# pszenher/Distributional_RL_Decision_and_Control

Hardware: AMD Instinct MI355X
Metric: env-steps/sec/GPU @4096 envs; IQN learn-steps/sec at 1/2/4/8 GPUs (higher is better)
Workload: dtype f64-env/bf16-learner; 1 GPU; BASELINE config 2: 4096 envs x 5 robots, 4 buoys, 55m map; fused rollout + AC-IQN learn (B=4096, N=N'=32) per step; envs_per_gpu=4096, robots=5, obstacles=4, global_batch=4096, num_tau=32, parallelism=dp1, hip_graphs=True, dp_rehearsal=False, unroll=2, chained=True, fused_reset=True, env_groups=0, target_after_env=False, push_after_actor=True, target_in_fused=True

## Files before the change

distributional_rl_decision_and_control_amd/_abi.py:

```python
import ctypes as C
import os

import numpy as np

HERE = os.path.dirname(os.path.abspath(__file__))
LIB_PATH = os.environ.get("ASVRL_LIB", os.path.join(HERE, "lib", "libasvrl.so"))
LIB_PATH_F32 = os.path.join(HERE, "lib", "libasvrl_f32.so")
OPERANDS = {"bf16": (LIB_PATH, 2), "f32": (LIB_PATH_F32, 4)}
ABI_VERSION = 29

SELF_DIM, OBJ_DIM, MAX_OBJ = 7, 5, 5
OBS_DIM = 40
TR_DIM = 88
PER_DIM = 48

F_X, F_Y, F_THETA, F_VR0, F_VR1, F_VR2, F_V0, F_V1, F_V2, F_TL, F_TR, F_LP, F_RP, F_GX, F_GY, F_PHI, F_RET = range(17)
NUM_FIELDS = 17

FLAG_DEACTIVATED, FLAG_COLLISION, FLAG_REACH_GOAL, FLAG_COLREGS = 1, 2, 4, 8

INFO_NORMAL, INFO_TOO_LONG, INFO_COLLISION, INFO_REACH_GOAL, INFO_DEACT_COLLISION, INFO_DEACT_GOAL = range(6)
INFO_ABSENT = 255
INFO_STRINGS = {
    INFO_NORMAL: "normal",
# ... 339 lines not shown
    ("asvrl_linear_wgrad_vec_groups", _I32, [_I32]),
    ("asvrl_linear_wgrad_partial", C.c_int, [_VP, _I64, _VP, _I64, _I32, _I32, _I32, _VP, _I64, _VP, _VP]),
    ("asvrl_linear_wgrad_multi", C.c_int, [_VP, _I32, _VP, _VP]),
    ("asvrl_linear_wgrad_vec_partial", C.c_int, [_VP, _I64, _VP, _I64, _I32, _I32, _VP, _I64, _VP, _VP]),
    ("asvrl_small_wgrad_partial", C.c_int, [_VP, _I64, _VP, _I64, _I32, _I32, _I32, _VP, _I64, _VP, _VP]),
    ("asvrl_partial_sums", C.c_int, [_VP, _I32, _VP]),
    ("asvrl_partial_sums_norm", C.c_int, [_VP, _I32, _VP, _VP, _VP]),
    ("asvrl_partial_sums_norm_parts", _I32, [_VP, _I32]),
    ("asvrl_actor_grads_workspace", _I64, [_I32]),
    ("asvrl_actor_grads_counters", _I32, []),
    ("asvrl_actor_grads_norm_parts", _I32, []),
    ("asvrl_actor_grads", C.c_int, [C.POINTER(AsvActorGradIO), _VP]),
    ("asvrl_adam_step", C.c_int, [_VP, _VP, _VP, _VP, _I64, _VP, _F, _F, _F, _F, _F, _VP, _VP, _I32, _VP]),
    ("asvrl_adam_step_pack", C.c_int, [_VP, _VP, _VP, _VP, _I64, _VP, _F, _F, _F, _F, _F, _VP, _VP, _I32, _VP, _I32,
                                       _VP, _VP]),
    ("asvrl_linear_wgrad", C.c_int, [_VP, _I64, _VP, _I64, _I32, _I32, _I32, _VP, _VP, _I32, _VP, _I64, _VP]),
    ("asvrl_linear_wgrad_vec", C.c_int, [_VP, _I64, _VP, _I64, _I32, _I32, _VP, _VP, _I32, _VP, _I64, _VP]),
    ("asvrl_mlp_pack", C.c_int, [C.POINTER(AsvMlpSrc), C.POINTER(AsvMlpWeights), _VP]),
    ("asvrl_mlp_encode", C.c_int, [C.POINTER(AsvMlpWeights), C.POINTER(AsvMlpIO), _VP]),
    ("asvrl_actor_forward", C.c_int, [C.POINTER(AsvMlpWeights), C.POINTER(AsvMlpIO), _I32, _VP]),
    ("asvrl_actor_backward", C.c_int, [C.POINTER(AsvMlpWeights), C.POINTER(AsvMlpIO), _VP]),
    ("asvrl_learn_prologue", C.c_int, [C.POINTER(AsvSampleArgs), C.POINTER(AsvMlpWeights), C.POINTER(AsvMlpIO),
                                       C.POINTER(AsvMlpWeights), _VP, _VP]),
    ("asvrl_encoder_fold", C.c_int, [_VP, _VP, _VP, _VP, _VP, _VP, _I32, _VP]),
    ("asvrl_small_wgrad", C.c_int, [_VP, _I64, _VP, _I64, _I32, _I32, _I32, _VP, _VP, _I32, _VP, _I64, _VP]),
    ("asvrl_last_error", C.c_char_p, []),
    ("asvrl_abi_version", C.c_int, []),
    ("asvrl_operand_bytes", C.c_int32, []),
    ("asvrl_struct_sizes", None, [C.c_void_p]),
    ("asvrl_rollout_struct_size", _I64, []),
    ("asvrl_policy_rollout", C.c_int, [C.POINTER(AsvParams), C.POINTER(AsvEnvState), C.POINTER(AsvStepCtl),
                                       C.POINTER(AsvStepOut), C.POINTER(AsvRollout), C.POINTER(AsvPolicy),
                                       C.POINTER(AsvEnvLaunch), _VP]),
    ("asvrl_policy_struct_size", _I64, []),
    ("asvrl_env_rollout_ar", C.c_int, [C.POINTER(AsvParams), C.POINTER(AsvEnvState), C.POINTER(AsvStepCtl),
                                       C.POINTER(AsvStepOut), C.POINTER(AsvRollout), C.POINTER(AsvAutoReset),
                                       C.POINTER(AsvEnvLaunch), _VP]),
    ("asvrl_policy_rollout_ar", C.c_int, [C.POINTER(AsvParams), C.POINTER(AsvEnvState), C.POINTER(AsvStepCtl),
                                          C.POINTER(AsvStepOut), C.POINTER(AsvRollout), C.POINTER(AsvPolicy),
                                          C.POINTER(AsvAutoReset), C.POINTER(AsvEnvLaunch), _VP]),
    ("asvrl_autoreset_struct_size", _I64, []),
    ("asvrl_replay_push_window", C.c_int, [_VP, _VP, _VP, _VP, _I32, _I64, _VP, _VP, _I32, _I32, _VP, _VP, _I64, _VP,
                                           _VP, _VP, _VP, _I64, _VP]),
    ("asvrl_eval_metrics", C.c_int, [C.POINTER(AsvEvalMetrics), _VP]),
    ("asvrl_eval_metrics_struct_size", _I64, []),
    ("asvrl_dqn_pack", C.c_int, [C.POINTER(AsvMlpSrc), _VP, C.POINTER(AsvDqnWeights), _VP]),
# ... 130 lines not shown
```

distributional_rl_decision_and_control_amd/csrc/asvrl_mlp.hip:

```cpp
#include "asvrl_common.h"
#include "asvrl_mfma.h"
#include "asvrl_lds.h"
#include "asvrl_actor_tile.h"

namespace asvrl {
namespace {
using namespace atile;

template <int KS, int P>
__device__ __forceinline__ f32x16 wchain(const frag8* W, int base, int lane, const elem_t* img, const RowA<P>& RA) {
  f32x16 acc = f32x16{};
#pragma unroll
  for (int ks = 0; ks < KS; ++ks) acc = mfma(W[(base + ks) * 64 + lane], rowf(img, RA, 0, ks), acc);
  return acc;
}

constexpr int kMlpWaves = 4;

__global__ __launch_bounds__(kMlpWaves * 64) void encode_kernel(MlpArgs a) {
  const int lane = threadIdx.x & 63, h = lane >> 5, r = lane & 31;
  const int tile = blockIdx.x * kMlpWaves + (threadIdx.x >> 6);
  const AsvMlpIO& io = a.io;
  if (tile * 32 >= io.n) return;
  const int row = tile * 32 + r;
  const bool valid = row < io.n;
  const int rr = valid ? row : io.n - 1;
// ... 145 lines not shown
  for (int ks = 0; ks < kEnc / 16; ++ks) q.w1[ks] = W1[(w * 16 + ks) * 64 + lane];
#pragma unroll
  for (int ks = 0; ks < kHid / 16; ++ks) q.w2[ks] = W2[(w * 8 + ks) * 64 + lane];
}

__device__ __forceinline__ void bias16(const float* tab, int mb, int h, float (&b)[16]) {
  typedef float f4v __attribute__((ext_vector_type(4)));
#pragma unroll
  for (int k = 0; k < 4; ++k) {
    const f4v t = *reinterpret_cast<const f4v*>(tab + mb * 32 + 8 * k + 4 * h);
#pragma unroll
    for (int i = 0; i < 4; ++i) b[4 * k + i] = t[i];
  }
}

static_assert(kSelfF >= 32 && kObjF >= 32, "a 32-feature block spans at most two encoders");
__device__ __forceinline__ float obj_sel(int ob, const float (&mf)[kObjN]) {
  float f = 1.f;
#pragma unroll
  for (int o = 0; o < kObjN; ++o) f = ob == o ? mf[o] : f;
  return f;
}

template <int MODE, bool PRE = false>
__device__ __forceinline__ void actor_split_tile(const MlpArgs& a, ActorSplitLds& L, int tile, const float* x,
                                                 int64_t ldx, int xrow0, const SplitPre& pre = SplitPre{}) {
  const AsvMlpIO& io = a.io;
  const int lane = threadIdx.x & 63, w = __builtin_amdgcn_readfirstlane(threadIdx.x >> 6), h = lane >> 5,
            r = lane & 31;
  const int row = tile * 32 + r;
  const bool valid = row < io.n;
  const int rr = valid ? row : io.n - 1;
  {
    frag8 bx[2];
    float mk[kObjN];
    load_obs(x, ldx, xrow0 + (rr - tile * 32), h, bx, mk);
    PRO_STAMP(10);
    if (MODE == MLP_TRAIN && w == 0 && valid) {
#pragma unroll
      for (int ks = 0; ks < 2; ++ks)
        *reinterpret_cast<frag8*>(bp(io.xb) + static_cast<int64_t>(row) * kObsK + ks * 16 + 8 * h) = bx[ks];
    }
    const frag8* ENC = reinterpret_cast<const frag8*>(a.w.enc_frag);
    const RowA<kEnc> RA(r, h);
    float mf[kObjN];
#pragma unroll
    for (int o = 0; o < kObjN; ++o) mf[o] = mk[o] < 0.5f ? 0.f : 1.f;
#pragma unroll
    for (int q = 0; q < 2; ++q) {
      const int mb = 2 * w + q;
      float bb[16];
      bias16(L.bias + kSbEnc, mb, h, bb);
      const int m_lo = mb * 32;
      const int obA = m_lo < kSelfF ? -1 : obj_of(m_lo);
      const int lim = kSelfF + kObjF * (obA + 1) - m_lo - 4 * h;
      const float fA = obj_sel(obA, mf), fB = obj_sel(obA + 1, mf);
      f32x16 acc = f32x16{};
#pragma unroll
      for (int ks = 0; ks < 2; ++ks)
        acc = mfma(PRE ? pre.enc[2 * q + ks] : ENC[(mb * 2 + ks) * 64 + lane], bx[ks], acc);
#pragma unroll
      for (int s = 0; s < 2; ++s) {
        float v[8];
#pragma unroll
        for (int j = 0; j < 8; ++j) {
          const int g = 8 * s + j;
          v[j] = relu(acc[g] + bb[g]) * ((g & 3) + 8 * (g >> 2) < lim ? fA : fB);
        }
        rows(L.x0, RA, 0, 2 * mb + s, pack8(v));
        if constexpr (MODE == MLP_TRAIN)
          store16(valid ? bp(io.h0) + static_cast<int64_t>(row) * kEnc + mb * 32 + 16 * s : nullptr, v, h);
      }
      if (q == 0) PRO_STAMP(11);
    }
  }
  PRO_STAMP(5);
  __syncthreads();
  PRO_STAMP(6);
  {
    const frag8* W1 = reinterpret_cast<const frag8*>(a.w.w1_frag);
    const RowA<kEnc> RX(r, h);
    const RowA<kHid> RH(r, h);
    float bb[16];
    bias16(L.bias + kSbB1, w, h, bb);
    f32x16 acc = f32x16{};
    if constexpr (PRE) {
#pragma unroll
      for (int ks = 0; ks < kEnc / 16; ++ks) acc = mfma(pre.w1[ks], rowf(L.x0, RX, 0, ks), acc);
    } else {
      acc = wchain<kEnc / 16>(W1, w * 16, lane, L.x0, RX);
    }
#pragma unroll
    for (int s = 0; s < 2; ++s) {
      float v[8];
#pragma unroll
      for (int j = 0; j < 8; ++j) v[j] = relu(acc[8 * s + j] + bb[8 * s + j]);
      rows(L.h1, RH, 0, 2 * w + s, pack8(v));
      if constexpr (MODE == MLP_TRAIN)
        store16(valid ? bp(io.h1) + static_cast<int64_t>(row) * kHid + w * 32 + 16 * s : nullptr, v, h);
    }
  }
  PRO_STAMP(7);
  __syncthreads();
  {
    const frag8* W2 = reinterpret_cast<const frag8*>(a.w.w2_frag);
    const RowA<kHid> RH(r, h);
    float bb[16], wo0[16], wo1[16];
    bias16(L.bias + kSbB2, w, h, bb);
    bias16(L.bias + kSbWout, w, h, wo0);
    bias16(L.bias + kSbWout + kHid, w, h, wo1);
    f32x16 acc = f32x16{};
    if constexpr (PRE) {
#pragma unroll
      for (int ks = 0; ks < kHid / 16; ++ks) acc = mfma(pre.w2[ks], rowf(L.h1, RH, 0, ks), acc);
    } else {
      acc = wchain<kHid / 16>(W2, w * 8, lane, L.h1, RH);
    }
    float p0 = 0.f, p1 = 0.f;
#pragma unroll
    for (int s = 0; s < 2; ++s) {
      float v[8];
#pragma unroll
      for (int j = 0; j < 8; ++j) {
        v[j] = relu(acc[8 * s + j] + bb[8 * s + j]);
        p0 += wo0[8 * s + j] * v[j];
        p1 += wo1[8 * s + j] * v[j];
      }
// ... 27 lines not shown
template <int MODE>
__global__ __launch_bounds__(kMlpWaves * 64) void actor_split_kernel(MlpArgs a) {
  __shared__ __attribute__((aligned(16))) ActorSplitLds L;
  SplitPre pre;
  split_prefetch(a.w, threadIdx.x >> 6, threadIdx.x & 63, pre);
  float bv[4];
  split_bias_fetch(a.w, threadIdx.x, bv);
  split_bias_store(L, threadIdx.x, bv);
  __syncthreads();
  actor_split_tile<MODE, true>(a, L, blockIdx.x, a.io.x, a.io.ldx, blockIdx.x * 32, pre);
}

struct PrologueArgs {
  const float* ring;
  int64_t cap;
  const int64_t* ring_state;
  uint64_t seed, counter;
  const uint64_t* counter_dev;
  int64_t guard;
  int B, tau_sets, tau_n;
  float* out;
  float* taus;
};

__global__ __launch_bounds__(kMlpWaves * 64) void learn_prologue_kernel(PrologueArgs p, MlpArgs train, MlpArgs tgt) {
  PRO_STAMP(0);
  __shared__ __attribute__((aligned(16))) ActorSplitLds L;
  __shared__ __attribute__((aligned(16))) float xs[32 * ASVRL_OBS_DIM];
  const int T = p.B / 32;
  const bool second = static_cast<int>(blockIdx.x) >= T;
  const int tile = second ? blockIdx.x - T : blockIdx.x;
  const int lane = threadIdx.x & 63, w = threadIdx.x >> 6;
  SplitPre pre;
  split_prefetch(second ? tgt.w : train.w, w, lane, pre);
  float bv[4];
  split_bias_fetch(second ? tgt.w : train.w, threadIdx.x, bv);
  const int64_t head = p.ring_state[0], size = p.ring_state[1];
  const uint64_t ctr = p.counter + (p.counter_dev != nullptr ? *p.counter_dev : 0ull);
  const int64_t my_slot = replay_draw_slot(head, size, p.cap, p.guard, tile * 32 + 8 * w + (lane & 7), p.seed, ctr);
  const int slot_lo = static_cast<int>(my_slot & 0xFFFFFFFFll), slot_hi = static_cast<int>(my_slot >> 32);
  PRO_STAMP(1);
  constexpr int kRowV = ASVRL_TR_DIM / 4, kObsV = ASVRL_OBS_DIM / 4;
  const int per = second ? kObsV : kRowV;
  typedef float f4v __attribute__((ext_vector_type(4)));
  f4v v[3];
  int jj[3], cc[3];
#pragma unroll
  for (int u = 0; u < 3; ++u) {
    const int e = lane + 64 * u;
    jj[u] = e / per;
    cc[u] = e - jj[u] * per;
    const int js = jj[u] < 8 ? jj[u] : 0;
    const int64_t slot = (static_cast<int64_t>(__shfl(slot_hi, js)) << 32) |
                         static_cast<uint32_t>(__shfl(slot_lo, js));
    v[u] = reinterpret_cast<const f4v*>(p.ring + slot * ASVRL_TR_DIM)[(second ? kObsV : 0) + (jj[u] < 8 ? cc[u] : 0)];
  }
  PRO_STAMP(2);
  if (!second && p.taus != nullptr) {
    const int per_row = p.tau_sets * p.tau_n, nblk = (per_row + 3) / 4;
    for (int it = lane; it < 8 * nblk; it += kWave) {
      const int j = it / nblk, k0 = 4 * (it - j * nblk), b = tile * 32 + 8 * w + j;
      const U4 r = philox4x32_10(U4{static_cast<uint32_t>(b), static_cast<uint32_t>(k0) ^ 0x7A0000u,
                                    static_cast<uint32_t>(ctr >> 32), static_cast<uint32_t>(ctr)},
                                 static_cast<uint32_t>(p.seed) ^ 0x51EDu, static_cast<uint32_t>(p.seed >> 32));
      const uint32_t rw[4] = {r.x, r.y, r.z, r.w};
#pragma unroll
      for (int q = 0; q < 4; ++q) {
        const int k = k0 + q;
        if (k < per_row) {
          const int set = k / p.tau_n, t = k - set * p.tau_n;
          p.taus[(static_cast<size_t>(set) * p.B + b) * p.tau_n + t] = static_cast<float>(rw[q] >> 8) * (1.0f / 16777216.0f);
        }
      }
    }
  }
#pragma unroll
  for (int u = 0; u < 3; ++u) {
    if (jj[u] < 8) {
      const int lr = 8 * w + jj[u], b = tile * 32 + lr;
      if (!second) reinterpret_cast<f4v*>(p.out + static_cast<size_t>(b) * ASVRL_TR_DIM)[cc[u]] = v[u];
      if (cc[u] < kObsV) reinterpret_cast<f4v*>(xs + lr * ASVRL_OBS_DIM)[cc[u]] = v[u];
    }
  }
  split_bias_store(L, threadIdx.x, bv);
  __syncthreads();
  PRO_STAMP(3);
  if (!second) actor_split_tile<MLP_TRAIN, true>(train, L, tile, xs, ASVRL_OBS_DIM, 0, pre);
  else actor_split_tile<MLP_FWD, true>(tgt, L, tile, xs, ASVRL_OBS_DIM, 0, pre);
  PRO_STAMP(4);
}

__device__ __forceinline__ void load_block16(const elem_t* rowp, int mb, int h, float (&v)[16]) {
#pragma unroll
  for (int g = 0; g < 16; g += 4) {
    float t[4];
    load4(rowp + mb * 32 + (g & 3) + 8 * (g >> 2) + 4 * h, t);
#pragma unroll
    for (int i = 0; i < 4; ++i) v[g + i] = t[i];
  }
}

__global__ __launch_bounds__(kMlpWaves * 64) void actor_bwd_split_kernel(MlpArgs a) {
  __shared__ __attribute__((aligned(16))) ActorSplitLds L;
  const AsvMlpIO& io = a.io;
  const int lane = threadIdx.x & 63, w = threadIdx.x >> 6, h = lane >> 5, r = lane & 31;
  const int row = blockIdx.x * 32 + r;
  const bool valid = row < io.n;
  const int64_t rr = valid ? row : io.n - 1;
  elem_t* const dz2i = L.x0;
  elem_t* const dz1i = L.h1;
  frag8 w2t[kHid / 16], w1t[2][kHid / 16];
  {
// ... 209 lines not shown
                                    const AsvMlpWeights* target_actor, float* na, void* stream) {
  ASVRL_REQUIRE(s && actor && train_io && target_actor && na && s->ring && s->ring_state && s->out,
                "asvrl_learn_prologue: null argument");
  ASVRL_REQUIRE(s->capacity > 0 && s->B > 0 && s->B % 32 == 0, "asvrl_learn_prologue: B must be a positive multiple of 32");
  ASVRL_REQUIRE(s->taus == nullptr || (s->tau_sets >= 1 && s->tau_n >= 1), "asvrl_learn_prologue: bad tau shape");
  ASVRL_REQUIRE(train_io->n == s->B && train_io->a_out && train_io->xb && train_io->h0 && train_io->h1 && train_io->h2 &&
                    train_io->pre, "asvrl_learn_prologue: the TRAIN outputs (n = B, a_out, xb, h0, h1, h2, pre)");
  for (const AsvMlpWeights* w : {actor, target_actor})
    ASVRL_REQUIRE(w->enc_frag && w->w1_frag && w->w2_frag && w->b1 && w->b2 && w->wout && w->bout,
                  "asvrl_learn_prologue: null actor weight");
  PrologueArgs p{s->ring, s->capacity, s->ring_state, s->seed, s->counter, s->counter_dev, s->guard,
                 s->B, s->tau_sets, s->tau_n, s->out, s->taus};
  MlpArgs tr{*actor, *train_io};
  AsvMlpIO fio{};
  fio.n = s->B;
  fio.a_out = na;
  fio.ld_aout = 2;
  MlpArgs tg{*target_actor, fio};
  hipLaunchKernelGGL(learn_prologue_kernel, dim3(2 * (s->B / 32)), dim3(kMlpWaves * 64), 0, as_stream(stream), p, tr,
                     tg);
  return check_launch("asvrl_learn_prologue");
}

extern "C" int asvrl_actor_backward(const AsvMlpWeights* w, const AsvMlpIO* io, void* stream) {
  ASVRL_REQUIRE(w && io && w->w2t_frag && w->w1t_frag && w->wout && io->dA && io->pre && io->h0 && io->h1 &&
                    io->h2 && io->dout && io->dz2 && io->dz1 && io->dz0,
                "asvrl_actor_backward: null argument");
  if (io->n <= 0) return 0;
  MlpArgs a{*w, *io};
  const int tiles = (io->n + 31) / 32;
  hipLaunchKernelGGL(actor_bwd_split_kernel, dim3(tiles), dim3(kMlpWaves * 64), 0, as_stream(stream), a);
  return check_launch("asvrl_actor_backward");
}

extern "C" int asvrl_encoder_fold(const float* dw, const float* db, float* self_w, float* self_b, float* obj_w,
                                  float* obj_b, int32_t accumulate, void* stream) {
  ASVRL_REQUIRE(dw && db && self_w && self_b && obj_w && obj_b, "asvrl_encoder_fold: null argument");
  const int n = kSelfF * kSelfIn + kObjF * kObjIn + kSelfF + kObjF;
  hipLaunchKernelGGL(enc_fold_kernel, dim3((n + 255) / 256), dim3(256), 0, as_stream(stream), dw, db, self_w,
                     self_b, obj_w, obj_b, accumulate);
  return check_launch("asvrl_encoder_fold");
}

extern "C" int asvrl_small_wgrad_partial(const float* dz, int64_t ldz, const float* x, int64_t ldx, int32_t R,
                                         int32_t M, int32_t K, float* partial, int64_t partial_floats,
                                         int32_t* groups_out, void* stream) {
// ... 22 lines not shown
```

distributional_rl_decision_and_control_amd/fused_update.py:

```python
import ctypes as C

import torch

from . import _abi
from .fused_critic import CriticPack, PartialArena, critic_actor_grad, critic_forward, critic_train_fused
from .fused_mlp import (ActorBuffers, ActorGrads, MlpPack, actor_act, actor_backward, actor_forward,
                        actor_train_forward)
from .fused_mlp import actor_grads as actor_grads_launch
from .learner import FusedAdam, clip_and_step

OBS = 40
ENC_IN_KERNEL = True
TARGET_IN_FUSED = True


def supported(policy, B, N):
    c, a = policy.critic, policy.actor
    return (c.concat_feature_dimension == 256 and c.hidden_dimension == 128 and c.n == 64 and N in (8, 16, 32)
            and (B * N) % 32 == 0 and B % 32 == 0 and c.self_dimension == 7 and c.object_dimension == 5
            and c.max_object_num == 5 and c.self_feature_dimension == 56 and c.object_feature_dimension == 40
            and a.hidden_dimension == 128 and a.concat_feature_dimension == 256 and a.action_dimension == 2
            and c.action_dimension == 2)


# ... 1 lines not shown

    def __init__(self, policy_local, policy_target, B, N, operands="bf16", double_actor=False):
        dev = policy_local.critic.cos_embedding.weight.device
        self.B, self.N, self.device = B, N, dev
        self.operands = operands
        self.local_trunk = CriticPack(policy_local.critic, operands)
        self.target_trunk = CriticPack(policy_target.critic, operands)
        self.actor = self.actor_pack = self.policy_pack = MlpPack(policy_local.actor, "actor", operands,
                                                                  double=double_actor)
        self.target_actor = MlpPack(policy_target.actor, "actor", operands)
        self.abufs = ActorBuffers(B, dev, operands)
        self.agrads = ActorGrads(B, dev, operands)
        f = dict(dtype=torch.float32, device=dev)
        bf = dict(dtype=_abi.operand_dtype(operands), device=dev)
        self.na = torch.empty(B, 2, **f)
        self.xb = torch.empty(B, 32, **bf)
        self.q_next = torch.empty(B * N, **f)
        self.q_pi = torch.empty(B * N, **f)
        self.dzF = torch.empty(B, 256, **bf)
        self.dzG = torch.empty(B, 128, **f)
        self.arena = PartialArena(32 << 20, dev, operands)
        self.losses = torch.zeros(2, **f)
        self.tile_loss = torch.zeros(2, B * N // 32, **f)

    def target_changed(self):
        self.target_trunk.refresh()
        self.target_actor.refresh()

    def refresh_local(self):
        self.local_trunk.refresh()
        self.actor.refresh()

    def act(self, obs_rows, actions64, step_dev, steps_per_count, total, fraction, initial, final, seed):
        actor_act(self.actor, obs_rows, actions64, step_dev, steps_per_count, total, fraction, initial, final, seed)

    def learn(self, tr, state=None, guard=0, actor_wait=None, target_wait=None, actor_done=None):
        rows = learn_prologue(self, tr.replay, tr.taus, tr.seed + 777, counter_dev=tr.learn_counter,
                              out=tr.batch_rows, state=state, guard=guard)
        return ac_iqn_update_fused2(self, tr.local, tr.actor_opt, tr.critic_opt, tr.critic_grads, tr.actor_grads,
                                    rows, gamma=tr.gamma, sync=tr.sync, actor_wait=actor_wait, taus=tr.taus,
                                    counter=tr.learn_counter, prologue_done=True, target_wait=target_wait,
                                    actor_done=actor_done)


def _reduce_and_step(arena, opt, grads, sync, max_norm, wait=None, pack=None, counter=None):
    assert pack is None or not isinstance(opt, FusedAdam) or opt.L is pack.L, "optimiser and pack of different builds"
    if isinstance(opt, FusedAdam):
        assert opt.max_norm == max_norm, (opt.max_norm, max_norm)
        if pack is not None and not hasattr(pack, "_adam_segs"):
            pack._adam_segs = pack.adam_segments(opt)
        segs = pack._adam_segs if pack is not None else None
        if sync is None:
            arena.flush(norm=opt)
            if wait is not None:
                torch.cuda.current_stream().wait_event(wait)
            return opt.step_prenormed(arena.norm_parts, arena.nparts, pack=segs, counter=counter)
        arena.flush()
        sync(grads)
        if wait is not None:
            torch.cuda.current_stream().wait_event(wait)
        return opt.step_synced(pack=segs, counter=counter)
    gn = _step_unfused(arena, opt, grads, sync, max_norm, wait)
    if pack is not None:
        pack.refresh()
    if counter is not None:
# ... 27 lines not shown
            agn = actor_opt.step_synced(pack=st.actor.adam_segments(actor_opt), counter=counter)
        st.actor.flip()
        return agn
    if sync is not None:
        sync(actor_grads)
    if actor_wait is not None:
        torch.cuda.current_stream().wait_event(actor_wait)
    agn = clip_and_step(actor_opt, actor_grads, max_norm)
    st.actor.refresh()
    if counter is not None:
        counter += 1
    return agn


def target_q(st, rows, tau0, q_out, na):
    ns_rows = rows[:, OBS:2 * OBS]
    actor_forward(st.target_actor, ns_rows, na)
    critic_forward(st.target_trunk, None, None, tau0, st.N, q=q_out, obs=ns_rows, act=na)


def learn_prologue(st, replay, taus, seed, counter_dev=None, counter=0, out=None, state=None, guard=0, stream=None):
    B = st.B
    out = out if out is not None else torch.empty((B, 88), dtype=torch.float32, device=st.device)
    sa = _abi.AsvSampleArgs()
    sa.ring, sa.capacity = replay.ring.data_ptr(), replay.capacity
    sa.ring_state = (state if state is not None else replay.state).data_ptr()
    sa.seed, sa.counter = int(seed) & 0xFFFFFFFFFFFFFFFF, int(counter) & 0xFFFFFFFFFFFFFFFF
    sa.counter_dev = _abi.ptr(counter_dev)
    sa.guard, sa.B, sa.out = int(guard), B, out.data_ptr()
    if taus is not None:
        assert taus.is_contiguous() and taus.shape[1] == B and taus.dtype == torch.float32
        sa.tau_sets, sa.tau_n, sa.taus = taus.shape[0], taus.shape[2], taus.data_ptr()
    io = st.abufs.io()
    _abi.check(st.actor.L.asvrl_learn_prologue(C.byref(sa), C.byref(st.actor.w), C.byref(io),
                                                C.byref(st.target_actor.w), st.na.data_ptr(),
                                                _abi.stream_ptr(stream)), "asvrl_learn_prologue", st.actor.L)
    return out


def ac_iqn_update_fused2(st, policy_local, actor_opt, critic_opt, critic_grads, actor_grads, rows, gamma=0.99,
                         taus=None, sync=None, max_norm=0.5, actor_wait=None, counter=None, prologue_done=False,
                         target_wait=None, actor_done=None):
    B, N = st.B, st.N
    critic, actor = policy_local.critic, policy_local.actor
    if taus is None:
        taus = torch.rand(3, B, N, device=st.device)
    s_rows = rows[:, 0:OBS]
    a_rows, r_col, d_col = rows[:, 80:82], rows[:, 82], rows[:, 83]
    ab, arena = st.abufs, st.arena

    q_next = st.q_next
    if target_wait is not None:
        torch.cuda.current_stream().wait_event(target_wait)
    target_in = TARGET_IN_FUSED and prologue_done and ENC_IN_KERNEL
    if target_in:
        pass
    elif prologue_done:
        critic_forward(st.target_trunk, None, None, taus[0], st.N, q=q_next, obs=rows[:, OBS:2 * OBS], act=st.na)
    else:
        actor_train_forward(st.actor, s_rows, ab)
        target_q(st, rows, taus[0], q_next, st.na)
    ae = critic.action_encoder[0]
    if ENC_IN_KERNEL:
        critic_train_fused(st.local_trunk, critic, taus[1], N, q_next.view(B, N), r_col, d_col, gamma, s_rows,
                           a_rows, arena, tile_loss=st.tile_loss[0], encoders=True,
                           target=(st.target_trunk, taus[0], rows[:, OBS:2 * OBS], st.na) if target_in else None)
    else:
        critic_train_fused(st.local_trunk, critic, taus[1], N, q_next.view(B, N), r_col, d_col, gamma, s_rows,
                           a_rows, arena, dzF=st.dzF, dzG=st.dzG, xb=st.xb, tile_loss=st.tile_loss[0])
        with arena.batch():
            arena.fold(st.dzF, st.xb, critic)
            arena.small(st.dzG, a_rows, ae.weight.grad, ae.bias.grad)
    arena.scalar(st.tile_loss[0], st.losses[0:1])
    cgn = _reduce_and_step(arena, critic_opt, critic_grads, sync, max_norm, pack=st.local_trunk)

    critic_actor_grad(st.local_trunk, None, None, taus[2], N, st.q_pi, w_ae=ae.weight, dA=ab.dA,
                      tile_loss=st.tile_loss[1], obs=s_rows, act=ab.a_out)
    if actor_done is not None:
# ... 5 lines not shown
```

distributional_rl_decision_and_control_amd/vec_trainer.py:

```python
import time

import torch

from . import streams
from .learn_ops import DevicePER, DeviceReplay
from .learner import FusedAdam
from .learners import LEARNERS, policy_modules, policy_parameters
from .vec_env import VecMarineNavEnv

DEFAULT_NET = dict(self_dimension=7, object_dimension=5, max_object_num=5, self_feature_dimension=56,
                   object_feature_dimension=40, concat_feature_dimension=256, hidden_dimension=128)


class VecTrainer:
    def __init__(self, n_envs=4096, agent_type="AC-IQN", num_robots=5, num_obs=4, num_cores=0, min_start_goal_dis=40.0,
                 width=55.0, batch_size=4096, num_tau=32, buffer_size=4_000_000, lr=1e-4, gamma=0.99,
                 learning_starts=None, target_update_interval=2500, total_timesteps=6_000_000,
                 exploration_fraction=0.25, initial_eps=0.6, final_eps=0.05, seed=0,
                 device="cuda", sync=None, graphs=False, schedule=None, net_seed=100, overlap=True, unroll=1,
                 chain=None, operands="bf16", target_after_env=False, push_after_actor=None):
        if agent_type not in LEARNERS:
            raise NotImplementedError(f"VecTrainer agent_type {agent_type!r} (AC-IQN, IQN, Rainbow, DQN and DDPG are "
                                      "batched)")
        spec = LEARNERS[agent_type]
        self.device = torch.device(device)
        self.agent_type = agent_type
        self.target_after_env = bool(target_after_env)
# ... 173 lines not shown
                actions=torch.zeros((K, NT, 2), dtype=torch.float64, device=dev),
                steps_run=torch.zeros(self.E, dtype=torch.int32, device=dev),
                pushed=torch.zeros(K, dtype=torch.int32, device=dev),
                resets=torch.zeros(self.E, dtype=torch.int32, device=dev))
        return bufs[K]

    @torch.no_grad()
    def collect(self, K, snap=None):
        if self.learner.actor_pack is None or self.per is not None:
            raise NotImplementedError("collect runs the AC-IQN / DDPG actor and pushes into the uniform ring; IQN, "
                                      "Rainbow and DQN act inside their own kernels")
        K = int(K)
        buf = self._collect_buffers(K)
        buf["obj_cnt"].fill_(-1)
        keep = {k: buf[k] for k in ("obs", "obs_prev", "obj_cnt", "reward", "done", "actions", "steps_run")}
        rec = self.env.policy_rollout(self.learner.actor_pack, K, hold_done=False, keep=keep,
                                      eps=(self.E, self.total_timesteps, self.exploration_fraction, self.initial_eps,
                                           self.final_eps), policy_seed=self.seed + 4242,
                                      auto_reset=dict(pushed=buf["pushed"], resets=buf["resets"]), count=False)
        self.replay.push_window(buf, K, pushed=buf["pushed"], snap=snap, counter_inc=self.env.counter, counter_by=K)
        self.env.advance_device(True)
        return rec

    def learn(self, state=None, guard=0, actor_wait=None, target_wait=None, actor_done=None):
        return self.learner.learn(self, state, guard, actor_wait, target_wait, actor_done)

    def hard_update(self):
        with torch.no_grad():
            torch._foreach_copy_(policy_parameters(self.target), policy_parameters(self.local))
            self.learner.target_changed()

    @torch.no_grad()
    def load_policies(self, local, target):
        assert self._graph is None, "load_policies before the first captured iteration"
        for dst, src in ((self.local, local), (self.target, target)):
            for d, s in zip(policy_modules(dst), policy_modules(src)):
                sd = s.state_dict()
                for name, t in d.state_dict(keep_vars=True).items():
                    t.data.copy_(sd[name].to(device=t.device, dtype=t.dtype))
        self.learner.refresh_local()
        self.learner.target_changed()

    def _iteration_body(self, do_learn):
        if not (do_learn and self.overlap and self.per is None):
            self.rollout()
            return self.learn() if do_learn else None
        main = torch.cuda.current_stream(self.device)
# ... 36 lines not shown
            self.learn_steps += 1
            if self.learn_steps % self.target_update_interval == 0:
                self.hard_update()
        self.last_losses = out
        return out

    def replay_size_host(self):
        if getattr(self, "_replay_ready", False):
            return self.learning_starts
        n = self.per.pushed if self.per is not None else self.replay.size()
        if n >= self.learning_starts:
            self._replay_ready = True
        return n

    def roll_stream(self):
        return streams.stream(self.device, "roll")

    def _roll_events(self):
        return torch.cuda.Event(), torch.cuda.Event()

    def _chained(self):
        return self.chain and self.overlap and self.per is None and self.unroll % 2 == 0

    def _chain_body(self):
        main = torch.cuda.current_stream(self.device)
        if self._streams is None:
            self._streams = (self.roll_stream(),) + self._roll_events()
        s_roll = self._streams[0]
        U = self.unroll
        ev_act = [torch.cuda.Event() for _ in range(U)]
        ev_snap = [torch.cuda.Event() for _ in range(U)]
        ev_learn = [torch.cuda.Event() for _ in range(U)]
        ev_env = [torch.cuda.Event() for _ in range(U)]
        ev_actor = [torch.cuda.Event() for _ in range(U)]
        self._chain_events = (ev_act, ev_snap, ev_learn, ev_env, ev_actor)
        tae, paa = self.target_after_env, self.push_after_actor
        s_roll.wait_stream(main)
        out = None

        def push_reset(k):
            self._push(snap=self.ring_snap2[k % 2])
            ev_snap[k].record(s_roll)
            self.env.auto_reset(True)
            self.env.advance_device(True)

        for k in range(U):
            with torch.cuda.stream(s_roll):
                if k > 0:
                    s_roll.wait_event(ev_learn[k - 1])
                self.act()
                ev_act[k].record(s_roll)
                self.env.step(self.actions)
                if tae:
                    ev_env[k].record(s_roll)
                if not paa:
                    push_reset(k)
            if k > 0:
                main.wait_event(ev_snap[k - 1])
            out = self.learn(state=self.ring_snap2[(k - 1) % 2], guard=self.E * self.R, actor_wait=ev_act[k],
                             target_wait=ev_env[k] if tae else None, actor_done=ev_actor[k] if paa else None)
            ev_learn[k].record(main)
            if paa:
                with torch.cuda.stream(s_roll):
                    s_roll.wait_event(ev_actor[k])
                    push_reset(k)
        main.wait_stream(s_roll)
        return out

    def _capture(self):
        s = streams.stream(self.device, "warmup")
        s.wait_stream(torch.cuda.current_stream(self.device))
        with torch.cuda.stream(s):
            for _ in range(3):
                self._iteration_body(True)
                self.env.advance_host()
        torch.cuda.current_stream(self.device).wait_stream(s)
        g = torch.cuda.CUDAGraph()
        chained = self._chained()
        if chained:
            self.ring_snap2[(self.unroll - 1) % 2].copy_(self.replay.state)
        with torch.cuda.graph(g, stream=streams.capture_stream(self.device), capture_error_mode="thread_local"):
            if chained:
                self._graph_out = self._chain_body()
            else:
                for _ in range(self.unroll):
                    self._graph_out = self._iteration_body(True)
        self._graph = g

    def run(self, iterations):
        t0 = time.time()
        for _ in range(iterations):
            self.iteration()
        torch.cuda.synchronize(self.device)
        return time.time() - t0
```

include/asvrl.h:

```cpp
#ifndef ASVRL_H
#define ASVRL_H

#include <stddef.h>
#include <stdint.h>

#ifdef __cplusplus
extern "C" {
#endif

#define ASVRL_ABI_VERSION 29

#define ASVRL_SELF_DIM 7
#define ASVRL_OBJ_DIM 5
#define ASVRL_MAX_OBJ 5
#define ASVRL_OBS_DIM 40
#define ASVRL_TR_DIM 88
#define ASVRL_PER_DIM 48

enum AsvRobotField {
  ASVRL_F_X = 0, ASVRL_F_Y, ASVRL_F_THETA,
  ASVRL_F_VR0, ASVRL_F_VR1, ASVRL_F_VR2,
  ASVRL_F_V0, ASVRL_F_V1, ASVRL_F_V2,
  ASVRL_F_TL, ASVRL_F_TR, ASVRL_F_LP, ASVRL_F_RP,
  ASVRL_F_GX, ASVRL_F_GY,
// ... 592 lines not shown
  void* dz0;
  const int64_t* step_dev;
  double eps_steps_per_count;
  double eps_total, eps_fraction, eps_initial, eps_final;
  uint64_t seed;
} AsvMlpIO;

int asvrl_mlp_pack(const AsvMlpSrc* src, const AsvMlpWeights* w, void* stream);
int asvrl_mlp_encode(const AsvMlpWeights* w, const AsvMlpIO* io, void* stream);
int asvrl_actor_forward(const AsvMlpWeights* w, const AsvMlpIO* io, int32_t mode, void* stream);
typedef struct AsvSampleArgs {
  const float* ring;
  int64_t capacity;
  const int64_t* ring_state;
  uint64_t seed, counter;
  const uint64_t* counter_dev;
  int64_t guard;
  int32_t B, tau_sets, tau_n, _pad0;
  float* out;
  float* taus;
} AsvSampleArgs;
int asvrl_learn_prologue(const AsvSampleArgs* s, const AsvMlpWeights* actor, const AsvMlpIO* train_io,
                         const AsvMlpWeights* target_actor, float* na, void* stream);
int asvrl_actor_backward(const AsvMlpWeights* w, const AsvMlpIO* io, void* stream);
int asvrl_encoder_fold(const float* dw, const float* db, float* self_w, float* self_b, float* obj_w,
                       float* obj_b, int32_t accumulate, void* stream);
int asvrl_small_wgrad(const float* dz, int64_t ldz, const float* x, int64_t ldx, int32_t R, int32_t M,
                      int32_t K, float* dw, float* db, int32_t accumulate, float* work,
                      int64_t work_floats, void* stream);
int asvrl_small_wgrad_partial(const float* dz, int64_t ldz, const float* x, int64_t ldx, int32_t R,
                              int32_t M, int32_t K, float* partial, int64_t partial_floats,
                              int32_t* groups_out, void* stream);


typedef struct AsvPolicy {
  AsvMlpWeights w;
  const float* obs_in;
  const int64_t* step_dev;
  double eps_steps_per_count, eps_total, eps_fraction, eps_initial, eps_final;
  uint64_t seed;
  double* actions;
} AsvPolicy;

int asvrl_policy_rollout(const AsvParams* params, const AsvEnvState* state, const AsvStepCtl* ctl,
                         const AsvStepOut* last, const AsvRollout* ro, const AsvPolicy* pi,
                         const AsvEnvLaunch* launch , void* stream);
// ... 176 lines not shown
```

Measured before the change: 16.55 million env-steps/s.

## Draw next learn batch and compute target critic ahead on rollout stream

```diff
diff --git a/distributional_rl_decision_and_control_amd/_abi.py b/distributional_rl_decision_and_control_amd/_abi.py
--- a/distributional_rl_decision_and_control_amd/_abi.py
+++ b/distributional_rl_decision_and_control_amd/_abi.py
@@ -385,6 +385,8 @@
     ("asvrl_actor_backward", C.c_int, [C.POINTER(AsvMlpWeights), C.POINTER(AsvMlpIO), _VP]),
     ("asvrl_learn_prologue", C.c_int, [C.POINTER(AsvSampleArgs), C.POINTER(AsvMlpWeights), C.POINTER(AsvMlpIO),
                                        C.POINTER(AsvMlpWeights), _VP, _VP]),
+    ("asvrl_draw_target", C.c_int, [C.POINTER(AsvSampleArgs), C.POINTER(AsvMlpWeights), _VP,
+                                    C.POINTER(AsvCriticWeights), _VP, _VP]),
     ("asvrl_encoder_fold", C.c_int, [_VP, _VP, _VP, _VP, _VP, _VP, _I32, _VP]),
     ("asvrl_small_wgrad", C.c_int, [_VP, _I64, _VP, _I64, _I32, _I32, _I32, _VP, _VP, _I32, _VP, _I64, _VP]),
     ("asvrl_last_error", C.c_char_p, []),
diff --git a/distributional_rl_decision_and_control_amd/csrc/asvrl_mlp.hip b/distributional_rl_decision_and_control_amd/csrc/asvrl_mlp.hip
--- a/distributional_rl_decision_and_control_amd/csrc/asvrl_mlp.hip
+++ b/distributional_rl_decision_and_control_amd/csrc/asvrl_mlp.hip
@@ -2,6 +2,7 @@
 #include "asvrl_mfma.h"
 #include "asvrl_lds.h"
 #include "asvrl_actor_tile.h"
+#include "asvrl_critic_tile.h"
 
 namespace asvrl {
 namespace {
@@ -193,7 +194,7 @@
   return f;
 }
 
-template <int MODE, bool PRE = false>
+template <int MODE, bool PRE = false, bool XW = false>
 __device__ __forceinline__ void actor_split_tile(const MlpArgs& a, ActorSplitLds& L, int tile, const float* x,
                                                  int64_t ldx, int xrow0, const SplitPre& pre = SplitPre{}) {
   const AsvMlpIO& io = a.io;
@@ -202,7 +203,8 @@
   const int row = tile * 32 + r;
   const bool valid = row < io.n;
   const int rr = valid ? row : io.n - 1;
-  {
+  const bool mine = !XW || w < kMlpWaves;
+  if (mine) {
     frag8 bx[2];
     float mk[kObjN];
     load_obs(x, ldx, xrow0 + (rr - tile * 32), h, bx, mk);
@@ -248,7 +250,7 @@
   PRO_STAMP(5);
   __syncthreads();
   PRO_STAMP(6);
-  {
+  if (mine) {
     const frag8* W1 = reinterpret_cast<const frag8*>(a.w.w1_frag);
     const RowA<kEnc> RX(r, h);
     const RowA<kHid> RH(r, h);
@@ -273,7 +275,7 @@
   }
   PRO_STAMP(7);
   __syncthreads();
-  {
+  if (mine) {
     const frag8* W2 = reinterpret_cast<const frag8*>(a.w.w2_frag);
     const RowA<kHid> RH(r, h);
     float bb[16], wo0[16], wo1[16];
@@ -347,6 +349,57 @@
   float* out;
   float* taus;
 };
+
+__device__ __forceinline__ void prologue_draw(const PrologueArgs& p, int tile, int w, int lane, uint64_t ctr,
+                                              int64_t head, int64_t size, bool full_row, bool rows_out, int stage_lo,
+                                              float* xs) {
+  const int64_t my_slot = replay_draw_slot(head, size, p.cap, p.guard, tile * 32 + 8 * w + (lane & 7), p.seed, ctr);
+  const int slot_lo = static_cast<int>(my_slot & 0xFFFFFFFFll), slot_hi = static_cast<int>(my_slot >> 32);
+  PRO_STAMP(1);
+  constexpr int kRowV = ASVRL_TR_DIM / 4, kObsV = ASVRL_OBS_DIM / 4;
+  const int per = full_row ? kRowV : kObsV;
+  typedef float f4v __attribute__((ext_vector_type(4)));
+  f4v v[3];
+  int jj[3], cc[3];
+#pragma unroll
+  for (int u = 0; u < 3; ++u) {
+    const int e = lane + 64 * u;
+    jj[u] = e / per;
+    cc[u] = e - jj[u] * per;
+    const int js = jj[u] < 8 ? jj[u] : 0;
+    const int64_t slot = (static_cast<int64_t>(__shfl(slot_hi, js)) << 32) |
+                         static_cast<uint32_t>(__shfl(slot_lo, js));
+    v[u] = reinterpret_cast<const f4v*>(p.ring + slot * ASVRL_TR_DIM)[(full_row ? 0 : kObsV) + (jj[u] < 8 ? cc[u] : 0)];
+  }
+  PRO_STAMP(2);
+  if (rows_out && p.taus != nullptr) {
+    const int per_row = p.tau_sets * p.tau_n, nblk = (per_row + 3) / 4;
+    for (int it = lane; it < 8 * nblk; it += kWave) {
+      const int j = it / nblk, k0 = 4 * (it - j * nblk), b = tile * 32 + 8 * w + j;
+      const U4 r = philox4x32_10(U4{static_cast<uint32_t>(b), static_cast<uint32_t>(k0) ^ 0x7A0000u,
+                                    static_cast<uint32_t>(ctr >> 32), static_cast<uint32_t>(ctr)},
+                                 static_cast<uint32_t>(p.seed) ^ 0x51EDu, static_cast<uint32_t>(p.seed >> 32));
+      const uint32_t rw[4] = {r.x, r.y, r.z, r.w};
+#pragma unroll
+      for (int q = 0; q < 4; ++q) {
+        const int k = k0 + q;
+        if (k < per_row) {
+          const int set = k / p.tau_n, t = k - set * p.tau_n;
+          p.taus[(static_cast<size_t>(set) * p.B + b) * p.tau_n + t] = static_cast<float>(rw[q] >> 8) * (1.0f / 16777216.0f);
+        }
+      }
+    }
+  }
+#pragma unroll
+  for (int u = 0; u < 3; ++u) {
+    if (jj[u] < 8) {
+      const int lr = 8 * w + jj[u], b = tile * 32 + lr;
+      if (rows_out) reinterpret_cast<f4v*>(p.out + static_cast<size_t>(b) * ASVRL_TR_DIM)[cc[u]] = v[u];
+      const int sc = cc[u] - (full_row ? stage_lo : 0);
+      if (sc >= 0 && sc < kObsV) reinterpret_cast<f4v*>(xs + lr * ASVRL_OBS_DIM)[sc] = v[u];
+    }
+  }
+}
 
 __global__ __launch_bounds__(kMlpWaves * 64) void learn_prologue_kernel(PrologueArgs p, MlpArgs train, MlpArgs tgt) {
   PRO_STAMP(0);
@@ -362,57 +415,81 @@
   split_bias_fetch(second ? tgt.w : train.w, threadIdx.x, bv);
   const int64_t head = p.ring_state[0], size = p.ring_state[1];
   const uint64_t ctr = p.counter + (p.counter_dev != nullptr ? *p.counter_dev : 0ull);
-  const int64_t my_slot = replay_draw_slot(head, size, p.cap, p.guard, tile * 32 + 8 * w + (lane & 7), p.seed, ctr);
-  const int slot_lo = static_cast<int>(my_slot & 0xFFFFFFFFll), slot_hi = static_cast<int>(my_slot >> 32);
-  PRO_STAMP(1);
-  constexpr int kRowV = ASVRL_TR_DIM / 4, kObsV = ASVRL_OBS_DIM / 4;
-  const int per = second ? kObsV : kRowV;
-  typedef float f4v __attribute__((ext_vector_type(4)));
-  f4v v[3];
-  int jj[3], cc[3];
-#pragma unroll
-  for (int u = 0; u < 3; ++u) {
-    const int e = lane + 64 * u;
-    jj[u] = e / per;
-    cc[u] = e - jj[u] * per;
-    const int js = jj[u] < 8 ? jj[u] : 0;
-    const int64_t slot = (static_cast<int64_t>(__shfl(slot_hi, js)) << 32) |
-                         static_cast<uint32_t>(__shfl(slot_lo, js));
-    v[u] = reinterpret_cast<const f4v*>(p.ring + slot * ASVRL_TR_DIM)[(second ? kObsV : 0) + (jj[u] < 8 ? cc[u] : 0)];
-  }
-  PRO_STAMP(2);
-  if (!second && p.taus != nullptr) {
-    const int per_row = p.tau_sets * p.tau_n, nblk = (per_row + 3) / 4;
-    for (int it = lane; it < 8 * nblk; it += kWave) {
-      const int j = it / nblk, k0 = 4 * (it - j * nblk), b = tile * 32 + 8 * w + j;
-      const U4 r = philox4x32_10(U4{static_cast<uint32_t>(b), static_cast<uint32_t>(k0) ^ 0x7A0000u,
-                                    static_cast<uint32_t>(ctr >> 32), static_cast<uint32_t>(ctr)},
-                                 static_cast<uint32_t>(p.seed) ^ 0x51EDu, static_cast<uint32_t>(p.seed >> 32));
-      const uint32_t rw[4] = {r.x, r.y, r.z, r.w};
-#pragma unroll
-      for (int q = 0; q < 4; ++q) {
-        const int k = k0 + q;
-        if (k < per_row) {
-          const int set = k / p.tau_n, t = k - set * p.tau_n;
-          p.taus[(static_cast<size_t>(set) * p.B + b) * p.tau_n + t] = static_cast<float>(rw[q] >> 8) * (1.0f / 16777216.0f);
-        }
-      }
-    }
-  }
-#pragma unroll
-  for (int u = 0; u < 3; ++u) {
-    if (jj[u] < 8) {
-      const int lr = 8 * w + jj[u], b = tile * 32 + lr;
-      if (!second) reinterpret_cast<f4v*>(p.out + static_cast<size_t>(b) * ASVRL_TR_DIM)[cc[u]] = v[u];
-      if (cc[u] < kObsV) reinterpret_cast<f4v*>(xs + lr * ASVRL_OBS_DIM)[cc[u]] = v[u];
-    }
-  }
+  prologue_draw(p, tile, w, lane, ctr, head, size, !second, !second, 0, xs);
   split_bias_store(L, threadIdx.x, bv);
   __syncthreads();
   PRO_STAMP(3);
   if (!second) actor_split_tile<MLP_TRAIN, true>(train, L, tile, xs, ASVRL_OBS_DIM, 0, pre);
   else actor_split_tile<MLP_FWD, true>(tgt, L, tile, xs, ASVRL_OBS_DIM, 0, pre);
   PRO_STAMP(4);
+}
+
+template <int NT> constexpr int kDtWaves = NT == 32 ? 8 : 4;
+template <int NT>
+struct DtCriticLds {
+  ctile::CriticLds W;
+  float F[kDtWaves<NT> * (32 / NT) * ctile::kC];
+  float G[kDtWaves<NT> * (32 / NT) * ctile::kH];
+};
+struct DtActorLds {
+  ActorSplitLds L;
+  float xs[32 * ASVRL_OBS_DIM];
+};
+template <int NT>
+union DtLds {
+  DtActorLds a;
+  DtCriticLds<NT> c;
+};
+
+template <int NT>
+__global__ __launch_bounds__(kDtWaves<NT> * 64) void draw_target_kernel(PrologueArgs p, MlpArgs tgt, ctile::CriticArgs c) {
+  constexpr int W = kDtWaves<NT>, S = 32 / NT;
+  constexpr bool XW = W > kMlpWaves;
+  __shared__ __attribute__((aligned(16))) DtLds<NT> U;
+  static_assert(sizeof(U) <= 160 * 1024, "draw + target LDS image exceeds the CU's 160 KB");
+  const int tile = blockIdx.x, lane = threadIdx.x & 63, w = __builtin_amdgcn_readfirstlane(threadIdx.x >> 6);
+  SplitPre pre;
+  if (!XW || w < kMlpWaves) {
+    split_prefetch(tgt.w, w, lane, pre);
+    float bv[4];
+    split_bias_fetch(tgt.w, threadIdx.x, bv);
+    const int64_t head = p.ring_state[0], size = p.ring_state[1];
+    const uint64_t ctr = p.counter + (p.counter_dev != nullptr ? *p.counter_dev : 0ull);
+    prologue_draw(p, tile, w, lane, ctr, head, size, true, true, ASVRL_OBS_DIM / 4, U.a.xs);
+    split_bias_store(U.a.L, threadIdx.x, bv);
+  }
+  __syncthreads();
+  actor_split_tile<MLP_FWD, true, XW>(tgt, U.a.L, tile, U.a.xs, ASVRL_OBS_DIM, 0, pre);
+  __syncthreads();
+  auto& L = U.c.W;
+  if constexpr (kWeightsInLds) {
+    copy_frags<W * 64, ctile::kFragWC, 16>(L.wc, reinterpret_cast<const frag8*>(c.w.wc_frag), threadIdx.x);
+    copy_frags<W * 64, ctile::kFragW1, 16>(L.w1, reinterpret_cast<const frag8*>(c.w.w1_frag), threadIdx.x);
+    copy_frags<W * 64, ctile::kFragW2, 16>(L.w2, reinterpret_cast<const frag8*>(c.w.w2_frag), threadIdx.x);
+  }
+  for (int i = threadIdx.x; i < ctile::kC; i += W * 64) L.bc[i] = c.w.bc[i];
+  for (int i = threadIdx.x; i < ctile::kH; i += W * 64) {
+    L.b1[i] = c.w.b1[i];
+    L.b2[i] = c.w.b2[i];
+    L.wo[i] = c.w.wo[i];
+  }
+  __syncthreads();
+#pragma nounroll
+  for (int i = w; i < NT; i += W) {
+    const int ct = tile * NT + i;
+    int wv = w;
+    asm volatile("" : "+v"(wv));
+    float* Fw = U.c.F + wv * S * ctile::kC;
+    float* Gw = U.c.G + wv * S * ctile::kH;
+    ctile::stage_features<NT, true, false>(c, ct, lane, Fw, Gw);
+    __builtin_amdgcn_fence(__ATOMIC_RELEASE, "wavefront");
+    __builtin_amdgcn_wave_barrier();
+    __builtin_amdgcn_fence(__ATOMIC_ACQUIRE, "wavefront");
+    ctile::critic_tile<ctile::MODE_FWD, NT>(c, L, ct, lane, Fw, Gw);
+    __builtin_amdgcn_fence(__ATOMIC_RELEASE, "wavefront");
+    __builtin_amdgcn_wave_barrier();
+    __builtin_amdgcn_fence(__ATOMIC_ACQUIRE, "wavefront");
+  }
 }
 
 __device__ __forceinline__ void load_block16(const elem_t* rowp, int mb, int h, float (&v)[16]) {
@@ -668,6 +745,45 @@
   return check_launch("asvrl_learn_prologue");
 }
 
+extern "C" int asvrl_draw_target(const AsvSampleArgs* s, const AsvMlpWeights* target_actor, float* na,
+                                 const AsvCriticWeights* target_critic, float* q_next, void* stream) {
+  ASVRL_REQUIRE(s && target_actor && na && target_critic && q_next && s->ring && s->ring_state && s->out && s->taus,
+                "asvrl_draw_target: null argument");
+  ASVRL_REQUIRE(s->capacity > 0 && s->B > 0 && s->B % 32 == 0, "asvrl_draw_target: B must be a positive multiple of 32");
+  ASVRL_REQUIRE(s->tau_sets >= 1 && (s->tau_n == 8 || s->tau_n == 16 || s->tau_n == 32),
+                "asvrl_draw_target: tau_sets >= 1 and N in 8, 16, 32");
+  const AsvMlpWeights* aw = target_actor;
+  ASVRL_REQUIRE(aw->enc_frag && aw->b_enc && aw->w1_frag && aw->w2_frag && aw->b1 && aw->b2 && aw->wout && aw->bout,
+                "asvrl_draw_target: null actor weight");
+  const AsvCriticWeights* cw = target_critic;
+  ASVRL_REQUIRE(cw->wc_frag && cw->w1_frag && cw->w2_frag && cw->bc && cw->b1 && cw->b2 && cw->wo && cw->bo &&
+                    cw->self_w && cw->self_b && cw->obj_w && cw->obj_b && cw->ae_w && cw->ae_b,
+                "asvrl_draw_target: null critic weight");
+  PrologueArgs p{s->ring, s->capacity, s->ring_state, s->seed, s->counter, s->counter_dev, s->guard,
+                 s->B, s->tau_sets, s->tau_n, s->out, s->taus};
+  AsvMlpIO fio{};
+  fio.n = s->B;
+  fio.a_out = na;
+  fio.ld_aout = 2;
+  MlpArgs tg{*aw, fio};
+  AsvCriticIO cio{};
+  cio.obs = s->out + ASVRL_OBS_DIM;
+  cio.ld_obs = ASVRL_TR_DIM;
+  cio.act = na;
+  cio.ld_act = 2;
+  cio.taus = s->taus;
+  cio.B = s->B;
+  cio.N = s->tau_n;
+  cio.q = q_next;
+  const ctile::CriticArgs ca = ctile::make_args(cw, &cio);
+  hipStream_t st = as_stream(stream);
+  const dim3 grid(s->B / 32);
+  if (s->tau_n == 8) hipLaunchKernelGGL(draw_target_kernel<8>, grid, dim3(kDtWaves<8> * 64), 0, st, p, tg, ca);
+  else if (s->tau_n == 16) hipLaunchKernelGGL(draw_target_kernel<16>, grid, dim3(kDtWaves<16> * 64), 0, st, p, tg, ca);
+  else hipLaunchKernelGGL(draw_target_kernel<32>, grid, dim3(kDtWaves<32> * 64), 0, st, p, tg, ca);
+  return check_launch("asvrl_draw_target");
+}
+
 extern "C" int asvrl_actor_backward(const AsvMlpWeights* w, const AsvMlpIO* io, void* stream) {
   ASVRL_REQUIRE(w && io && w->w2t_frag && w->w1t_frag && w->wout && io->dA && io->pre && io->h0 && io->h1 &&
                     io->h2 && io->dout && io->dz2 && io->dz1 && io->dz0,
diff --git a/distributional_rl_decision_and_control_amd/fused_update.py b/distributional_rl_decision_and_control_amd/fused_update.py
--- a/distributional_rl_decision_and_control_amd/fused_update.py
+++ b/distributional_rl_decision_and_control_amd/fused_update.py
@@ -47,6 +47,22 @@
         self.arena = PartialArena(32 << 20, dev, operands)
         self.losses = torch.zeros(2, **f)
         self.tile_loss = torch.zeros(2, B * N // 32, **f)
+        self.inputs = None
+
+    def enable_target_ahead(self, tr):
+        if self.inputs is None:
+            B, N, f = self.B, self.N, dict(dtype=torch.float32, device=self.device)
+            self.inputs = [LearnInputs(tr.batch_rows, tr.taus, self.na, self.q_next),
+                           LearnInputs(torch.zeros_like(tr.batch_rows), torch.zeros_like(tr.taus),
+                                       torch.empty(B, 2, **f), torch.empty(B * N, **f))]
+            self.draw_base = torch.zeros(1, dtype=torch.int64, device=self.device)
+
+    def draw_target(self, tr, k, state, guard, stream=None):
+        s = self.inputs[k % 2]
+        sa = _sample_args(self, tr.replay, s.taus, tr.seed + 777, self.draw_base, k, s.rows, state, guard)
+        _abi.check(self.actor.L.asvrl_draw_target(C.byref(sa), C.byref(self.target_actor.w), s.na.data_ptr(),
+                                                  C.byref(self.target_trunk.struct), s.q_next.data_ptr(),
+                                                  _abi.stream_ptr(stream)), "asvrl_draw_target", self.actor.L)
 
     def target_changed(self):
         self.target_trunk.refresh()
@@ -59,13 +75,38 @@
     def act(self, obs_rows, actions64, step_dev, steps_per_count, total, fraction, initial, final, seed):
         actor_act(self.actor, obs_rows, actions64, step_dev, steps_per_count, total, fraction, initial, final, seed)
 
-    def learn(self, tr, state=None, guard=0, actor_wait=None, target_wait=None, actor_done=None):
-        rows = learn_prologue(self, tr.replay, tr.taus, tr.seed + 777, counter_dev=tr.learn_counter,
-                              out=tr.batch_rows, state=state, guard=guard)
+    def learn(self, tr, state=None, guard=0, actor_wait=None, target_wait=None, actor_done=None, ahead=None):
+        if ahead is not None:
+            s = self.inputs[ahead % 2]
+            actor_train_forward(self.actor, s.rows[:, 0:OBS], self.abufs)
+            rows, taus = s.rows, s.taus
+        else:
+            s, taus = None, tr.taus
+            rows = learn_prologue(self, tr.replay, tr.taus, tr.seed + 777, counter_dev=tr.learn_counter,
+                                  out=tr.batch_rows, state=state, guard=guard)
         return ac_iqn_update_fused2(self, tr.local, tr.actor_opt, tr.critic_opt, tr.critic_grads, tr.actor_grads,
-                                    rows, gamma=tr.gamma, sync=tr.sync, actor_wait=actor_wait, taus=tr.taus,
+                                    rows, gamma=tr.gamma, sync=tr.sync, actor_wait=actor_wait, taus=taus,
                                     counter=tr.learn_counter, prologue_done=True, target_wait=target_wait,
-                                    actor_done=actor_done)
+                                    actor_done=actor_done, q_next=s.q_next if s is not None else None)
+
+
+class LearnInputs:
+
+    def __init__(self, rows, taus, na, q_next):
+        self.rows, self.taus, self.na, self.q_next = rows, taus, na, q_next
+
+
+def _sample_args(st, replay, taus, seed, counter_dev, counter, out, state, guard):
+    sa = _abi.AsvSampleArgs()
+    sa.ring, sa.capacity = replay.ring.data_ptr(), replay.capacity
+    sa.ring_state = (state if state is not None else replay.state).data_ptr()
+    sa.seed, sa.counter = int(seed) & 0xFFFFFFFFFFFFFFFF, int(counter) & 0xFFFFFFFFFFFFFFFF
+    sa.counter_dev = _abi.ptr(counter_dev)
+    sa.guard, sa.B, sa.out = int(guard), st.B, out.data_ptr()
+    if taus is not None:
+        assert taus.is_contiguous() and taus.shape[1] == st.B and taus.dtype == torch.float32
+        sa.tau_sets, sa.tau_n, sa.taus = taus.shape[0], taus.shape[2], taus.data_ptr()
+    return sa
 
 
 def _reduce_and_step(arena, opt, grads, sync, max_norm, wait=None, pack=None, counter=None):
@@ -139,15 +180,7 @@
 def learn_prologue(st, replay, taus, seed, counter_dev=None, counter=0, out=None, state=None, guard=0, stream=None):
     B = st.B
     out = out if out is not None else torch.empty((B, 88), dtype=torch.float32, device=st.device)
-    sa = _abi.AsvSampleArgs()
-    sa.ring, sa.capacity = replay.ring.data_ptr(), replay.capacity
-    sa.ring_state = (state if state is not None else replay.state).data_ptr()
-    sa.seed, sa.counter = int(seed) & 0xFFFFFFFFFFFFFFFF, int(counter) & 0xFFFFFFFFFFFFFFFF
-    sa.counter_dev = _abi.ptr(counter_dev)
-    sa.guard, sa.B, sa.out = int(guard), B, out.data_ptr()
-    if taus is not None:
-        assert taus.is_contiguous() and taus.shape[1] == B and taus.dtype == torch.float32
-        sa.tau_sets, sa.tau_n, sa.taus = taus.shape[0], taus.shape[2], taus.data_ptr()
+    sa = _sample_args(st, replay, taus, seed, counter_dev, counter, out, state, guard)
     io = st.abufs.io()
     _abi.check(st.actor.L.asvrl_learn_prologue(C.byref(sa), C.byref(st.actor.w), C.byref(io),
                                                 C.byref(st.target_actor.w), st.na.data_ptr(),
@@ -157,7 +190,7 @@
 
 def ac_iqn_update_fused2(st, policy_local, actor_opt, critic_opt, critic_grads, actor_grads, rows, gamma=0.99,
                          taus=None, sync=None, max_norm=0.5, actor_wait=None, counter=None, prologue_done=False,
-                         target_wait=None, actor_done=None):
+                         target_wait=None, actor_done=None, q_next=None):
     B, N = st.B, st.N
     critic, actor = policy_local.critic, policy_local.actor
     if taus is None:
@@ -166,11 +199,12 @@
     a_rows, r_col, d_col = rows[:, 80:82], rows[:, 82], rows[:, 83]
     ab, arena = st.abufs, st.arena
 
-    q_next = st.q_next
+    target_done = q_next is not None
+    q_next = q_next if target_done else st.q_next
     if target_wait is not None:
         torch.cuda.current_stream().wait_event(target_wait)
-    target_in = TARGET_IN_FUSED and prologue_done and ENC_IN_KERNEL
-    if target_in:
+    target_in = TARGET_IN_FUSED and prologue_done and ENC_IN_KERNEL and not target_done
+    if target_in or target_done:
         pass
     elif prologue_done:
         critic_forward(st.target_trunk, None, None, taus[0], st.N, q=q_next, obs=rows[:, OBS:2 * OBS], act=st.na)
diff --git a/distributional_rl_decision_and_control_amd/vec_trainer.py b/distributional_rl_decision_and_control_amd/vec_trainer.py
--- a/distributional_rl_decision_and_control_amd/vec_trainer.py
+++ b/distributional_rl_decision_and_control_amd/vec_trainer.py
@@ -2,7 +2,7 @@
 
 import torch
 
-from . import streams
+from . import fused_update, streams
 from .learn_ops import DevicePER, DeviceReplay
 from .learner import FusedAdam
 from .learners import LEARNERS, policy_modules, policy_parameters
@@ -222,7 +222,9 @@
         self.env.advance_device(True)
         return rec
 
-    def learn(self, state=None, guard=0, actor_wait=None, target_wait=None, actor_done=None):
+    def learn(self, state=None, guard=0, actor_wait=None, target_wait=None, actor_done=None, ahead=None):
+        if ahead is not None:
+            return self.learner.learn(self, state, guard, actor_wait, target_wait, actor_done, ahead=ahead)
         return self.learner.learn(self, state, guard, actor_wait, target_wait, actor_done)
 
     def hard_update(self):
@@ -305,6 +307,10 @@
     def _chained(self):
         return self.chain and self.overlap and self.per is None and self.unroll % 2 == 0
 
+    def _target_ahead(self):
+        return (self.agent_type == "AC-IQN" and self.graphs and self._chained() and self.operands == "bf16"
+                and fused_update.TARGET_IN_FUSED and fused_update.ENC_IN_KERNEL and not self.target_after_env)
+
     def _chain_body(self):
         main = torch.cuda.current_stream(self.device)
         if self._streams is None:
@@ -316,14 +322,25 @@
         ev_learn = [torch.cuda.Event() for _ in range(U)]
         ev_env = [torch.cuda.Event() for _ in range(U)]
         ev_actor = [torch.cuda.Event() for _ in range(U)]
-        self._chain_events = (ev_act, ev_snap, ev_learn, ev_env, ev_actor)
+        ev_tgt = [torch.cuda.Event() for _ in range(U)]
+        self._chain_events = (ev_act, ev_snap, ev_learn, ev_env, ev_actor, ev_tgt)
         tae, paa = self.target_after_env, self.push_after_actor
+        ahead = self._target_ahead()
         s_roll.wait_stream(main)
+        if ahead:
+            with torch.cuda.stream(s_roll):
+                self.learner.draw_base.copy_(self.learn_counter)
         out = None
-
-        def push_reset(k):
+        early_push = ahead or not paa
+
+        def push(k):
             self._push(snap=self.ring_snap2[k % 2])
             ev_snap[k].record(s_roll)
+            if ahead and k + 1 < U:
+                self.learner.draw_target(self, k + 1, self.ring_snap2[k % 2], self.E * self.R)
+                ev_tgt[k + 1].record(s_roll)
+
+        def reset():
             self.env.auto_reset(True)
             self.env.advance_device(True)
 
@@ -336,17 +353,22 @@
                 self.env.step(self.actions)
                 if tae:
                     ev_env[k].record(s_roll)
+                if early_push:
+                    push(k)
                 if not paa:
-                    push_reset(k)
+                    reset()
             if k > 0:
-                main.wait_event(ev_snap[k - 1])
+                main.wait_event(ev_tgt[k] if ahead else ev_snap[k - 1])
             out = self.learn(state=self.ring_snap2[(k - 1) % 2], guard=self.E * self.R, actor_wait=ev_act[k],
-                             target_wait=ev_env[k] if tae else None, actor_done=ev_actor[k] if paa else None)
+                             target_wait=ev_env[k] if tae else None, actor_done=ev_actor[k] if paa else None,
+                             ahead=k if ahead and k > 0 else None)
             ev_learn[k].record(main)
             if paa:
                 with torch.cuda.stream(s_roll):
                     s_roll.wait_event(ev_actor[k])
-                    push_reset(k)
+                    if not early_push:
+                        push(k)
+                    reset()
         main.wait_stream(s_roll)
         return out
 
@@ -362,6 +384,8 @@
         chained = self._chained()
         if chained:
             self.ring_snap2[(self.unroll - 1) % 2].copy_(self.replay.state)
+            if self._target_ahead():
+                self.learner.enable_target_ahead(self)
         with torch.cuda.graph(g, stream=streams.capture_stream(self.device), capture_error_mode="thread_local"):
             if chained:
                 self._graph_out = self._chain_body()
diff --git a/include/asvrl.h b/include/asvrl.h
--- a/include/asvrl.h
+++ b/include/asvrl.h
@@ -638,6 +638,8 @@
 } AsvSampleArgs;
 int asvrl_learn_prologue(const AsvSampleArgs* s, const AsvMlpWeights* actor, const AsvMlpIO* train_io,
                          const AsvMlpWeights* target_actor, float* na, void* stream);
+int asvrl_draw_target(const AsvSampleArgs* s, const AsvMlpWeights* target_actor, float* na,
+                      const AsvCriticWeights* target_critic, float* q_next, void* stream);
 int asvrl_actor_backward(const AsvMlpWeights* w, const AsvMlpIO* io, void* stream);
 int asvrl_encoder_fold(const float* dw, const float* db, float* self_w, float* self_b, float* obj_w,
                        float* obj_b, int32_t accumulate, void* stream);
```

Result: slower. 16.29 million env-steps/s (-1.6%).
